# CelestineAngla/BundleAdjustment.jl

Hardware: AMD Instinct MI355X
Metric: LM iterations/sec on BAL venice-1778 (synthetic BAL-shaped), plus Jacobian Mnnz/sec (higher is better)
Workload: dtype f64; 1 GPU; venice-1778 shape: ncams=1778 npnts=993923 nobs=5001946, seed 20261004, lm.jl variant, LDL/None, facto_type f64, fixed 83 iterations, perm AMD; parallelism=points sharded over 1 rank(s), cameras replicated

## Files before the change

### bundleadjustment.jl_amd/csrc/ba_dense_ldl.hip

```cpp
#include "ba_internal.h"

#include <algorithm>
#include <atomic>
#include <cmath>
#include <cstdio>
#include <cstdlib>

namespace {

template <typename T>
struct RT;
template <>
struct RT<double> {
  typedef double v4 __attribute__((ext_vector_type(4)));
  typedef double v2 __attribute__((ext_vector_type(2)));
  static __device__ inline v4 mfma(double a, double b, v4 c) { return __builtin_amdgcn_mfma_f64_16x16x4f64(a, b, c, 0, 0, 0); }
  static __device__ inline int row(int lane, int reg) { return (lane >> 4) + 4 * reg; }
};
template <>
struct RT<float> {
  typedef float v4 __attribute__((ext_vector_type(4)));
  typedef float v2 __attribute__((ext_vector_type(2)));
  static __device__ inline v4 mfma(float a, float b, v4 c) { return __builtin_amdgcn_mfma_f32_16x16x4f32(a, b, c, 0, 0, 0); }
  static __device__ inline int row(int lane, int reg) { return 4 * (lane >> 4) + reg; }
// ... 965 lines not shown
    const int col = wc + 16 * n + (lane & 15);
    const T inv_d = (T)1 / Dk[col];
#pragma unroll
    for (int m = 0; m < 4; m++)
#pragma unroll
      for (int g = 0; g < 4; g++) {
        const int row = wr + 16 * m + RT<T>::row(lane, g);
        const T xv = acc[m][n][g];
        V10[row * NB + col] = xv;
        S10[row * NB + col] = xv * inv_d;
      }
  }
  __threadfence();
  __syncthreads();
  if (FWD) {
    if (tid < NB) {
      T sacc = 0;
      for (int c = 0; c < NB; c++) sacc += S10[tid * NB + c] * ysh[c];
      b[(int64_t)(k + 1) * NB + tid] -= sacc;
    }
  }
#pragma unroll
  for (int m = 0; m < 4; m++)
#pragma unroll
    for (int n = 0; n < 4; n++) acc[m][n] = (d4){0, 0, 0, 0};
  tile_gemm_abt<T, 1>(V10, S10, nullptr, nullptr, sm, sm + NB * LDK, acc);
#pragma unroll
  for (int n = 0; n < 4; n++) {
    const int col = wc + 16 * n + (lane & 15);
#pragma unroll
    for (int m = 0; m < 4; m++)
#pragma unroll
      for (int g = 0; g < 4; g++) {
        const int row = wr + 16 * m + RT<T>::row(lane, g);
        S11[row * NB + col] -= acc[m][n][g];
      }
  }
  __threadfence();
  __syncthreads();
  T *Lk1 = Lk + NB * NB, *Dk1 = Dk + NB;
  diag_tile<T, 4>(S11, Lk1, Dk1, flag, nullptr, sm);
  if (FWD) {
    __threadfence();
    __syncthreads();
    if (tid < NB) {
      T sacc = 0;
      for (int c = 0; c <= tid; c++) sacc += Lk1[tid * NB + c] * b[(int64_t)(k + 1) * NB + c];
      y[(int64_t)(k + 1) * NB + tid] = sacc;
    }
  }
}

template <typename T>
__device__ __forceinline__ void ldl_update_tile(T *__restrict__ S, const int64_t *__restrict__ co, const T *__restrict__ V0, const T *__restrict__ V1,
                                       int k, int i, int j, T *lds, const T *__restrict__ Lp0, const T *__restrict__ Lp1) {
  BA_VT
  T *Sij = S + tix(co, i, j) * NB * NB;
  typename RT<T>::v4 acc[4][4];
#pragma unroll
  for (int m = 0; m < 4; m++)
#pragma unroll
    for (int n = 0; n < 4; n++) acc[m][n] = (d4){0, 0, 0, 0};
  tile_gemm_abt_priv<T, 2>(V0 + (int64_t)i * NB * NB, Lp0 ? Lp0 + (int64_t)j * NB * NB : S + tix(co, j, k) * NB * NB,
                        V1 + (int64_t)i * NB * NB, Lp1 ? Lp1 + (int64_t)j * NB * NB : S + tix(co, j, k + 1) * NB * NB, lds, acc);
  int tid2 = threadIdx.x;
  asm volatile("" : "+v"(tid2));
  const int lane = tid2 & 63, wv = (tid2 >> 6) & 3;
  const int wr = (wv >> 1) * 64, wc = (wv & 1) * 64;
  T *cbase = Sij + wr * NB + wc + (lane & 15);
#pragma unroll
  for (int h = 0; h < 2; h++) {
    T cv[2][4][4];
#pragma unroll
    for (int n2 = 0; n2 < 2; n2++)
#pragma unroll
      for (int m = 0; m < 4; m++)
#pragma unroll
        for (int g = 0; g < 4; g++) cv[n2][m][g] = cbase[(16 * m + RT<T>::row(lane, g)) * NB + 16 * (2 * h + n2)];
#pragma unroll
    for (int n2 = 0; n2 < 2; n2++)
#pragma unroll
      for (int m = 0; m < 4; m++)
#pragma unroll
        for (int g = 0; g < 4; g++) {
          const T nv = cv[n2][m][g] - acc[m][2 * h + n2][g];
          cbase[(16 * m + RT<T>::row(lane, g)) * NB + 16 * (2 * h + n2)] = nv;
        }
  }
}

template <typename T, int MODE, bool OWN = false>
__global__ __launch_bounds__(256, 2) void k_ldl_update(T *__restrict__ S, const int64_t *__restrict__ co, const T *__restrict__ V0,
                                                        const T *__restrict__ V1, int k, int base, int nt,
                                                        int nblk, int *__restrict__ ready,
                                                        const int *__restrict__ own_cols = nullptr,
                                                        const int64_t *__restrict__ own_pref = nullptr, int m0 = 0,
                                                        int m_end = 0, int ready_tiles = 1, const int *__restrict__ rows = nullptr,
                                                        const T *__restrict__ Lp0 = nullptr, const T *__restrict__ Lp1 = nullptr,
                                                        const int2 *__restrict__ tlist = nullptr, int blocked = TSB) {
  BA_VT
  static_assert(MODE == 1, "only the pair update is a tile-per-workgroup kernel");
  extern __shared__ __attribute__((aligned(16))) unsigned char smraw[];
  T *lds = reinterpret_cast<T *>(smraw);
  int i, j, tsel;
  {
    const int per = (nblk + 7) / 8;
    int t = (blockIdx.x & 7) * per + (blockIdx.x >> 3);
    if (t >= nblk) return;
    tsel = t;
    if (tlist) {
      i = tlist[t].x;
      j = tlist[t].y;
    } else if (OWN) {
      const int64_t tt = t + own_pref[m0];
      int lo = m0, hi = m_end;
      while (hi - lo > 1) {
        const int mid = (lo + hi) >> 1;
        if (own_pref[mid] <= tt) lo = mid;
        else hi = mid;
      }
      j = own_cols[lo];
      i = j + (int)(tt - own_pref[lo]);
    } else {
      int m_rows = (int)((sqrt(8.0 * (double)nblk + 1.0) - 1.0) * 0.5);
      while ((m_rows + 1) * (m_rows + 2) / 2 <= nblk) m_rows++;
      while (m_rows * (m_rows + 1) / 2 > nblk) m_rows--;
      int ii, jj;
      if (blocked) {
        tri_blocked(t, m_rows, &ii, &jj, blocked);
      } else {
        ii = (int)((sqrt(8.0 * (double)t + 1.0) - 1.0) * 0.5);
        while ((ii + 1) * (ii + 2) / 2 <= t) ii++;
        while (ii * (ii + 1) / 2 > t) ii--;
        jj = t - ii * (ii + 1) / 2;
      }
      i = rows ? rows[ii] : base + ii;
      j = rows ? rows[jj] : base + jj;
    }
  }
  ldl_update_tile<T>(S, co, V0, V1, k, i, j, lds, Lp0, Lp1);
  if (ready && tsel < ready_tiles) {
    __threadfence();
    __syncthreads();
    if (threadIdx.x == 0) __hip_atomic_fetch_add(ready, 1, __ATOMIC_RELEASE, __HIP_MEMORY_SCOPE_AGENT);
  }
}

template <typename T>
constexpr size_t part_lds_bytes() { return 2 * gemm_priv_lds_bytes<T>(); }
template <typename T>
__global__ __launch_bounds__(512) void k_ldl_update_part(T *__restrict__ S, const int64_t *__restrict__ co, const T *__restrict__ V0,
                                                          const T *__restrict__ V1, int k, int nblk, const int *__restrict__ rows) {
  extern __shared__ __attribute__((aligned(16))) unsigned char smraw[];
  const int half = __builtin_amdgcn_readfirstlane((int)(threadIdx.x >> 8));
  T *lds = reinterpret_cast<T *>(smraw + half * gemm_priv_lds_bytes<T>());
  for (int t = 2 * blockIdx.x + half; t < nblk; t += 2 * gridDim.x) {
    int ii = (int)((sqrt(8.0 * (double)t + 1.0) - 1.0) * 0.5);
    while ((ii + 1) * (ii + 2) / 2 <= t) ii++;
    while (ii * (ii + 1) / 2 > t) ii--;
    const int jj = t - ii * (ii + 1) / 2;
    ldl_update_tile<T>(S, co, V0, V1, k, rows[ii], rows[jj], lds, nullptr, nullptr);
  }
}

template <typename T>
__global__ __launch_bounds__(512) void k_ldl_update_part2(T *__restrict__ S, const int64_t *__restrict__ co, RunPanel<T> a, int nblk_a,
                                                           RunPanel<T> c, int nblk_c, int64_t panel) {
  extern __shared__ __attribute__((aligned(16))) unsigned char smraw[];
  const int half = __builtin_amdgcn_readfirstlane((int)(threadIdx.x >> 8));
  T *lds = reinterpret_cast<T *>(smraw + half * gemm_priv_lds_bytes<T>());
  for (int tt = 2 * blockIdx.x + half; tt < nblk_a + nblk_c; tt += 2 * gridDim.x) {
    const bool second = tt >= nblk_a;
    const RunPanel<T> &r = second ? c : a;
    const int t = tt - (second ? nblk_a : 0);
    int ii = (int)((sqrt(8.0 * (double)t + 1.0) - 1.0) * 0.5);
    while ((ii + 1) * (ii + 2) / 2 <= t) ii++;
    while (ii * (ii + 1) / 2 > t) ii--;
    const int jj = t - ii * (ii + 1) / 2;
    ldl_update_tile<T>(S, co, r.V, r.V + panel, r.k, r.rows[ii], r.rows[jj], lds, nullptr, nullptr);
  }
}

template <typename T>
__global__ __launch_bounds__(256, 2) void k_ldl_update2(T *__restrict__ S, const int64_t *__restrict__ co, RunPanel<T> a, int nblk_a,
                                                         RunPanel<T> c, int nblk_c, int64_t panel) {
  extern __shared__ __attribute__((aligned(16))) unsigned char smraw[];
  T *lds = reinterpret_cast<T *>(smraw);
  const int ga = ((nblk_a + 7) / 8) * 8;
  const bool second = (int)blockIdx.x >= ga;
  const RunPanel<T> &r = second ? c : a;
  const int nblk = second ? nblk_c : nblk_a, bid = (int)blockIdx.x - (second ? ga : 0);
  const int per = (nblk + 7) / 8;
  const int t = (bid & 7) * per + (bid >> 3);
  if (t >= nblk) return;
  int ii = (int)((sqrt(8.0 * (double)t + 1.0) - 1.0) * 0.5);
  while ((ii + 1) * (ii + 2) / 2 <= t) ii++;
  while (ii * (ii + 1) / 2 > t) ii--;
  const int jj = t - ii * (ii + 1) / 2;
  ldl_update_tile<T>(S, co, r.V, r.V + panel, r.k, r.rows[ii], r.rows[jj], lds, nullptr, nullptr);
}

template <typename T>
__global__ __launch_bounds__(256) void k_ldl_scale_panel(T *__restrict__ Lcol, const T *__restrict__ V, const T *__restrict__ D_k, int i0,
                                                          const int *__restrict__ rows = nullptr) {
  BA_VT
  const int i = rows ? rows[blockIdx.x] : i0 + blockIdx.x;
  const T *Vi = V + (int64_t)i * NB * NB;
  T *Sik = Lcol + (int64_t)i * NB * NB;
  const int c2 = threadIdx.x & 63;
  const T inv0 = (T)1 / D_k[2 * c2], inv1 = (T)1 / D_k[2 * c2 + 1];
  for (int r = threadIdx.x >> 6; r < NB; r += 4) {
    d2 v = *reinterpret_cast<const d2 *>(Vi + r * NB + 2 * c2);
    v.x *= inv0;
    v.y *= inv1;
// ... 254 lines not shown
  col_off->assign((size_t)nt, 0);
  if (own_range) own_range->assign((size_t)world + 1, 0);
  int64_t off = 0;
  for (int r = 0; r < world; r++) {
    if (own_range) (*own_range)[(size_t)r] = off;
    for (int64_t q = r; 2 * q < nt; q += world)
      for (int64_t j = 2 * q; j < 2 * q + 2 && j < nt; j++) {
        (*col_off)[(size_t)j] = off;
        off += nt - j;
      }
  }
  if (own_range) (*own_range)[(size_t)world] = off;
}

template <typename T>
int dense_ldl_alloc(DenseLDLT<T> *w, int64_t n_unpadded, int world, int rank, bool lazy_S, bool own_only) {
  int64_t nt = (n_unpadded + NB - 1) / NB;
  if (nt < 1) nt = 1;
  w->n = nt * NB;
  w->nt = nt;
  w->world = world;
  w->rank = rank;
  dense_ldl_layout(nt, world, &w->h_glob_off, &w->own_range);
  w->h_col_tab.assign((size_t)nt + 1, 0);
  for (int64_t j = 0; j < nt; j++) w->hco()[j] = w->h_glob_off[(size_t)j];
  w->own_only = own_only && world > 1;
  w->s_tiles = nt * (nt + 1) / 2;
  if (w->own_only) {
    const int64_t base = w->own_range[(size_t)rank];
    for (int64_t j = 0; j < nt; j++)
      w->hco()[j] = ((j / 2) % world == rank) ? w->hco()[j] - base : BA_NO_TILE;
    w->s_tiles = std::max<int64_t>(1, w->own_range[(size_t)rank + 1] - base);
  }
  BA_CHECK(upload(w->col_tab, w->h_col_tab));
  w->col_off = w->col_tab + 1;
  w->h_own_cols.clear();
  w->h_own_pref.assign(1, 0);
  for (int64_t j = 0; j < nt; j++)
    if ((j / 2) % world == rank) {
      w->h_own_cols.push_back((int)j);
      w->h_own_pref.push_back(w->h_own_pref.back() + (nt - j));
    }
  BA_CHECK(upload(w->own_cols, w->h_own_cols, 1));
  BA_CHECK(upload(w->own_pref, w->h_own_pref));
  BA_CHECK(w->flag_sum.alloc(1));
  if (!lazy_S) BA_CHECK(dense_ldl_alloc_S(w));
  BA_CHECK(w->ev_chain.create(hipEventDisableTiming | hipEventReleaseToDevice));
  BA_CHECK(w->Linv.alloc(nt * NB * NB));
  BA_HIP_CHECK(hipMemset(w->Linv, 0, (size_t)nt * NB * NB * sizeof(T)));
  BA_HIP_CHECK(hipDeviceSynchronize());
  BA_CHECK(w->D.alloc(nt * NB * 2));
  BA_CHECK(w->flag.alloc(1));
  BA_CHECK(w->ready.alloc(nt));
  BA_CHECK(w->hoist.create(hipStreamNonBlocking));
  {
    int lo = 0, hi = 0;
    BA_HIP_CHECK(hipDeviceGetStreamPriorityRange(&lo, &hi));
    BA_CHECK(w->rest.create(hipStreamNonBlocking, lo));
  }
  BA_CHECK(w->ev_top.create(hipEventDisableTiming | hipEventReleaseToDevice));
  BA_CHECK(w->ev_dtop.create(hipEventDisableTiming));
  BA_CHECK(w->ev_dchain.create(hipEventDisableTiming));
  for (int q = 0; q < 2; q++) {
    BA_CHECK(w->ev_recv[q].create(hipEventDisableTiming));
    BA_CHECK(w->ev_upd[q].create(hipEventDisableTiming));
  }
  return set_kernel_attrs<T>();
}

template <typename T>
int dense_ldl_alloc_S(DenseLDLT<T> *w) {
  if (!w->S) BA_CHECK(w->S.alloc(w->s_tiles * NB * NB));
  if (!w->V) BA_CHECK(w->V.alloc(8 * w->nt * NB * NB));
  if (!w->Lb && w->own_only) BA_CHECK(w->Lb.alloc(4 * w->nt * NB * NB));
  if (!w->bpart && w->own_only) BA_CHECK(w->bpart.alloc(2 * w->nt * NB));
  return BA_OK;
}

struct PairRows {
  int k, c1, c2;
  const int *rows1, *rows2;
  const int *h_rows1;
  int row(int a) const { return h_rows1 ? h_rows1[a] : k + 1 + a; }
};

template <typename T>
static PairRows pair_rows(const DenseLDLT<T> *w, int q) {
  PairRows r = {2 * q, 0, 0, nullptr, nullptr, nullptr};
  if (const TilePattern *pat = w->pat) {
    const int l0 = pat->prow_ptr[(size_t)q];
    r.c1 = pat->prow_ptr[(size_t)q + 1] - l0;
    r.rows1 = w->prow + l0;
    r.rows2 = r.rows1 + 1;
    r.h_rows1 = pat->prow.data() + l0;
  } else {
    r.c1 = std::max(0, (int)w->nt - r.k - 1);
  }
  r.c2 = r.c1 > 0 ? r.c1 - 1 : 0;
  return r;
}

template <typename T>
static int launch_diag(ba_problem *p, DenseLDLT<T> *w, int k, hipStream_t st, const int *wait_ready = nullptr, bool clear_flag = false) {
  ProfScope ps(p, PC_LDL_DIAG, st);
  hipLaunchKernelGGL(k_ldl_diag<T>, dim3(1), dim3(DIAG_THREADS), DIAG_LDS_ELEMS * sizeof(T), st, w->S + tix(w->hco(), k, k) * NB * NB,
                     w->Linv + (int64_t)k * NB * NB, w->D + (int64_t)k * NB, w->flag, (unsigned long long *)nullptr,
                     wait_ready, clear_flag ? 1 : 0);
  return BA_OK;
}

template <typename K>
static K fwd_kernel(const void *b, K with_fwd, K without) { return b ? with_fwd : without; }

template <typename T>
static int launch_trsm(ba_problem *p, DenseLDLT<T> *w, int k, const int *rows, int count, T *V, T *b, hipStream_t st) {
  T *y = w->D + w->nt * NB;
  if (count <= 0) {
    if (b) hipLaunchKernelGGL(k_fwd_step<T>, dim3(1), dim3(256), 0, st, w->S, w->col_off, w->Linv, b, y, k);
    return BA_OK;
  }
  ProfScope ps(p, PC_LDL_TRSM, st);
  hipLaunchKernelGGL(fwd_kernel(b, k_ldl_trsm_rs<T, true>, k_ldl_trsm_rs<T, false>), dim3(4 * count), dim3(256), RS_LDS_ELEMS * sizeof(T),
                     st, w->S, w->col_off, w->Linv + (int64_t)k * NB * NB, w->D + (int64_t)k * NB, V, k, b, y, rows);
  return BA_OK;
}

template <typename T>
static int launch_col(ba_problem *p, DenseLDLT<T> *w, int k, const int *rows, int count, const T *V0, hipStream_t st) {
  if (count <= 0) return BA_OK;
  ProfScope ps(p, PC_LDL_SYRK, st);
  hipLaunchKernelGGL(k_ldl_col_rs<T>, dim3(4 * count), dim3(256), RS_LDS_ELEMS * sizeof(T), st, w->S, w->col_off, V0, k, rows);
  return BA_OK;
}

static int update_rs_max() {
  return env_int("BA_LDL_UPDATE_RS_MAX", 320);
}

template <typename T>
static int launch_pair(ba_problem *p, DenseLDLT<T> *w, int k, const int *rows, int count, const T *V0, const T *V1, hipStream_t st,
                       int *ready = nullptr, int ready_tiles = 1) {
  const int nblk = count * (count + 1) / 2;
  if (nblk <= 0) return BA_OK;
  if (!ready && nblk <= update_rs_max()) {
    ProfScope ps(p, PC_LDL_UPDATE_RS, st);
    hipLaunchKernelGGL(k_ldl_update_rs<T>, dim3(4 * nblk), dim3(256), RS_LDS_ELEMS * sizeof(T), st, w->S, w->col_off, V0, V1, k, k + 2, nblk,
                       rows);
    return BA_OK;
  }
  ProfScope ps(p, PC_LDL_UPDATE, st);
  hipLaunchKernelGGL((k_ldl_update<T, 1>), dim3(((nblk + 7) / 8) * 8), dim3(256), gemm_priv_lds_bytes<T>(), st, w->S,
                     w->col_off, V0, V1, k, k + 2, (int)w->nt, nblk, ready, (const int *)nullptr, (const int64_t *)nullptr, 0, 0,
                     ready_tiles, rows);
  return BA_OK;
}

template <typename T>
static int launch_pairdiag(ba_problem *p, DenseLDLT<T> *w, int k, T *V0, T *b, hipStream_t st, const int *wait_ready, int need) {
  ProfScope ps(p, PC_LDL_DIAG, st);
  T *y = w->D + w->nt * NB;
  hipLaunchKernelGGL(fwd_kernel(b, k_ldl_pairdiag<T, true>, k_ldl_pairdiag<T, false>), dim3(1), dim3(256), DIAG_LDS_ELEMS * sizeof(T), st,
                     w->S, w->col_off, w->Linv, w->D, V0, k, (int)w->nt, w->flag, wait_ready, need, b, y);
  return BA_OK;
}

template <typename T>
static int launch_pairtrsm(ba_problem *p, DenseLDLT<T> *w, int k, T *V0, T *V1, T *b, hipStream_t st) {
  const int m = (int)w->nt - k - 2;
  if (m <= 0) return BA_OK;
  ProfScope ps(p, PC_LDL_TRSM, st);
  const T *y = w->D + w->nt * NB;
  hipLaunchKernelGGL(fwd_kernel(b, k_ldl_pairtrsm<T, true>, k_ldl_pairtrsm<T, false>), dim3(4 * m), dim3(256), PT_LDS_ELEMS * sizeof(T), st,
                     w->S, w->col_off, w->Linv, w->D, V0, V1, k, b, y);
  return BA_OK;
}

template <typename T>
static int panel_chain(ba_problem *p, DenseLDLT<T> *w, const PairRows &r, T *V0, T *V1, T *b, hipStream_t st) {
  launch_trsm(p, w, r.k, r.rows1, r.c1, V0, b, st);
  if (r.c1 == 0) return BA_OK;
  launch_col(p, w, r.k, r.rows1, r.c1, V0, st);
  launch_diag(p, w, r.k + 1, st);
  launch_trsm(p, w, r.k + 1, r.rows2, r.c2, V1, b, st);
  return BA_OK;
}

template <typename T>
int dense_ldl_factor_sparse(ba_problem *p, DenseLDLT<T> *w, hipStream_t st, T *d_b);

template <typename T>
int dense_ldl_factor(ba_problem *p, DenseLDLT<T> *w, hipStream_t st, T *d_b) {
  if (w->sparse && !p->comm.active()) return dense_ldl_factor_sparse(p, w, st, d_b);
  const int nt = (int)w->nt;
  static const bool hoist_off = env_off("BA_LDL_HOIST");
  w->hoisting = !p->prof_on && !hoist_off && !w->hoist_disabled && !p->comm.active() && nt >= HOIST_MIN_TILES + 2 && nt <= HOIST_MAX_TILES;
  if (w->hoisting) {
    BA_HIP_CHECK(hipMemsetAsync(w->flag, 0, sizeof(int), st));
    BA_HIP_CHECK(hipMemsetAsync(w->ready, 0, (size_t)nt * sizeof(int), st));
    BA_HIP_CHECK(hipEventRecord(w->ev_top, st));
    BA_HIP_CHECK(hipStreamWaitEvent(w->hoist, w->ev_top, 0));
  }
  constexpr int FUSE_MIN_TILES = 48;
  static const bool fuse_off = env_off("BA_LDL_FUSE");
  auto fused = [&](int k) { return w->hoisting && !fuse_off && k >= 2 && k + 1 < nt && nt - k >= FUSE_MIN_TILES; };
  launch_diag(p, w, 0, st, nullptr, !w->hoisting);
  for (int k = 0, slot = 0; k < nt; k += 2, slot ^= 1) {
    const PairRows r = pair_rows(w, k / 2);
    T *V0 = w->vpanel(slot, 0), *V1 = w->vpanel(slot, 1);
    const bool more = k + 2 < nt;
    const bool next_fused = more && fused(k + 2);
    const bool next_hoist1 = more && !next_fused && w->hoisting && (nt - k - 2 >= HOIST_MIN_TILES);
    const int need = (k + 3 < nt) ? 3 : 1;
    if (next_fused) {
      launch_pairdiag(p, w, k + 2, w->vpanel(slot ^ 1, 0), d_b, w->hoist, w->ready + k + 2, need);
      BA_HIP_CHECK(hipEventRecord(w->ev_chain, w->hoist));
    } else if (next_hoist1) {
      launch_diag(p, w, k + 2, w->hoist, w->ready + k + 2);
      BA_HIP_CHECK(hipEventRecord(w->ev_chain, w->hoist));
    }
    if (fused(k)) launch_pairtrsm(p, w, k, V0, V1, d_b, st);
    else panel_chain(p, w, r, V0, V1, d_b, st);
    if (!more) break;
    const bool hoisted = next_fused || next_hoist1;
    launch_pair(p, w, k, r.rows2, r.c2, V0, V1, st, hoisted ? w->ready + k + 2 : nullptr, next_fused ? need : 1);
    if (hoisted)
      BA_HIP_CHECK(hipStreamWaitEvent(st, w->ev_chain, 0));
    else
      launch_diag(p, w, k + 2, st);
  }
  BA_HIP_CHECK(hipGetLastError());
  return BA_OK;
}


template <typename T>
int dense_ldl_use_pattern(DenseLDLT<T> *w, const TilePattern *pat) {
  for (DevBuf<int> *q : {&w->prow, &w->lcol, &w->lpair}) q->reset();
  w->upd_ij.reset();
  w->own_tiles.reset();
  w->pat = pat;
  w->sparse = pat != nullptr;
  if (!pat) return BA_OK;
  {
    const int64_t nt = w->nt;
    const int P = w->own_only ? w->world : 1, me = w->own_only ? w->rank : 0;
    std::vector<int64_t> tab((size_t)(1 + nt + nt * nt), BA_NO_TILE);
    tab[0] = nt;
    int64_t *co = tab.data() + 1, *rp = tab.data() + 1 + nt;
    w->h_col_cnt.assign((size_t)nt, 0);
    for (int64_t j = 0; j < nt; j++) {
      const int64_t q = j / 2;
      int64_t pos = 0;
      rp[j * nt + j] = pos++;
      const int l0 = pat->prow_ptr[(size_t)q], l1 = pat->prow_ptr[(size_t)q + 1];
      for (int l = l0; l < l1; l++) {
        const int64_t i = pat->prow[(size_t)l];
        if (i > j) rp[i * nt + j] = pos++;
      }
      w->h_col_cnt[(size_t)j] = pos;
    }
    w->own_range.assign((size_t)P + 1, 0);
    int64_t run = 0;
    for (int r = 0; r < P; r++) {
      w->own_range[(size_t)r] = run;
      for (int64_t j = 0; j < nt; j++)
        if ((j / 2) % P == r) {
          if (r == me) co[j] = run;
          run += w->h_col_cnt[(size_t)j];
        }
    }
    w->own_range[(size_t)P] = run;
    const int64_t base = w->own_range[(size_t)me];
    for (int64_t j = 0; j < nt; j++)
      if (co[j] >= 0) co[j] -= base;
    w->s_tiles = std::max<int64_t>(1, w->own_range[(size_t)me + 1] - base);
    if (w->own_only) {
      w->h_own_pref.assign(1, 0);
      std::vector<int2> tiles;
      for (int j : w->h_own_cols) {
        w->h_own_pref.push_back(w->h_own_pref.back() + w->h_col_cnt[(size_t)j]);
        const int64_t q = j / 2;
        tiles.push_back(make_int2(j, j));
        for (int l = pat->prow_ptr[(size_t)q]; l < pat->prow_ptr[(size_t)q + 1]; l++)
          if (pat->prow[(size_t)l] > j) tiles.push_back(make_int2(pat->prow[(size_t)l], j));
      }
      BA_HIP_CHECK(hipMemcpy(w->own_pref, w->h_own_pref.data(), w->h_own_pref.size() * sizeof(int64_t), hipMemcpyHostToDevice));
      BA_CHECK(upload(w->own_tiles, tiles, 1));
      std::vector<int2> upd;
      const int npairs = (int)((nt + 1) / 2);
      w->h_upd_ptr.assign(1, 0);
      w->h_upd_lead.assign((size_t)npairs, 0);
      for (int q = 0; q < npairs; q++) {
        const int k = 2 * q, l0 = pat->prow_ptr[(size_t)q], l1 = pat->prow_ptr[(size_t)q + 1];
        for (int a = l0 + 1; a < l1; a++) {
          const int j = pat->prow[(size_t)a];
          if ((j / 2) % P != me) continue;
          for (int c = a; c < l1; c++) upd.push_back(make_int2(pat->prow[(size_t)c], j));
          if (j < k + 4) w->h_upd_lead[(size_t)q] = (int)upd.size() - w->h_upd_ptr.back();
        }
        w->h_upd_ptr.push_back((int)upd.size());
      }
      BA_CHECK(upload(w->upd_ij, upd, 1));
    }
    w->h_col_tab.swap(tab);
    BA_CHECK(upload(w->col_tab, w->h_col_tab));
    w->col_off = w->col_tab + 1;
    if (w->S) BA_CHECK(w->S.alloc(w->s_tiles * NB * NB));
  }
  BA_CHECK(upload(w->prow, pat->prow, 1));
  BA_CHECK(upload(w->lcol, pat->lcol, 1));
  BA_CHECK(upload(w->lpair, pat->lpair, 1));
  return BA_OK;
}

constexpr int REST_CUS = 224;
static int rest_grid(int ntile) { return (ntile + 1) / 2 < REST_CUS ? (ntile + 1) / 2 : REST_CUS; }

struct UpdateSplit {
  int nlead, lead_tiles, rest_tiles;
};
static UpdateSplit update_split(const PairRows &r) {
  int nlead = 0;
  while (nlead < r.c2 && nlead < 2 && r.row(1 + nlead) < r.k + 4) nlead++;
  const int nrest = r.c2 - nlead;
  return {nlead, nlead == 0 ? 0 : (nlead == 1 ? r.c2 : 2 * r.c2 - 1), nrest * (nrest + 1) / 2};
}

template <typename T>
int dense_ldl_factor_sparse(ba_problem *p, DenseLDLT<T> *w, hipStream_t st, T *d_b) {
  const int nt = (int)w->nt;
  const TilePattern *pat = w->pat;
  const int64_t panel = (int64_t)nt * NB * NB;
  const int npairs = (nt + 1) / 2;
  T *y = w->D + w->nt * NB;
  w->hoisting = false;
  const bool lookahead = !p->prof_on && !env_off("BA_SPARSE_LOOKAHEAD");
  const int la_min = env_int("BA_SPARSE_LOOKAHEAD_MIN", 96);
  bool pending[2] = {false, false};
  auto join_rest = [&](int slot) -> int {
    if (pending[slot]) {
      BA_HIP_CHECK(hipStreamWaitEvent(st, w->ev_upd[slot], 0));
      pending[slot] = false;
    }
    return BA_OK;
  };
  auto fork_rest = [&](int slot) -> int {
    BA_HIP_CHECK(hipEventRecord(w->ev_recv[slot], st));
    BA_HIP_CHECK(hipStreamWaitEvent(w->rest, w->ev_recv[slot], 0));
    return BA_OK;
  };
  auto rest_launched = [&](int slot) -> int {
    BA_HIP_CHECK(hipEventRecord(w->ev_upd[slot], w->rest));
    pending[slot] = true;
    return BA_OK;
  };
  const bool two = pat->a_clean > 0 && pat->b_clean > 0 && !p->prof_on && !env_off("BA_SPARSE_TWO_RUNS");
  std::vector<int> order;
  if (two) {
    BA_HIP_CHECK(hipMemsetAsync(w->flag, 0, sizeof(int), st));
    const int both = std::min(pat->a_clean, pat->b_clean);
    for (int i = 0; i < both; i++) {
      const int slot = i & 1;
      const PairRows a = pair_rows(w, i), b = pair_rows(w, pat->split + i);
      T *VA = w->vpanel(slot, 0, 0), *VB = w->vpanel(slot, 0, 1);
      auto tile = [&](int k) { return w->S + tix(w->hco(), k, k) * NB * NB; };
      auto panel_of = [&](int k, T *V, const int *rows) { return RunPanel<T>{w->Linv + (int64_t)k * NB * NB, w->D + (int64_t)k * NB, V, k, rows}; };
      auto diag2 = [&](int ka, int kb) {
        hipLaunchKernelGGL(k_ldl_diag2<T>, dim3(2), dim3(DIAG_THREADS), DIAG_LDS_ELEMS * sizeof(T), st, tile(ka), w->Linv + (int64_t)ka * NB * NB,
                           w->D + (int64_t)ka * NB, tile(kb), w->Linv + (int64_t)kb * NB * NB, w->D + (int64_t)kb * NB, w->flag);
      };
      auto trsm2 = [&](const RunPanel<T> &pa, int ca, const RunPanel<T> &pb, int cb) {
        hipLaunchKernelGGL(fwd_kernel(d_b, k_ldl_trsm_rs2<T, true>, k_ldl_trsm_rs2<T, false>), dim3(4 * (ca + cb)), dim3(256),
                           RS_LDS_ELEMS * sizeof(T), st, w->S, w->col_off, pa, pb, 4 * ca, d_b, y);
      };
      BA_CHECK(join_rest(slot));
      diag2(a.k, b.k);
      const RunPanel<T> a0 = panel_of(a.k, VA, a.rows1), b0 = panel_of(b.k, VB, b.rows1);
      trsm2(a0, a.c1, b0, b.c1);
      hipLaunchKernelGGL(k_ldl_col_rs2<T>, dim3(4 * (a.c1 + b.c1)), dim3(256), RS_LDS_ELEMS * sizeof(T), st, w->S, w->col_off, a0, b0, 4 * a.c1);
      diag2(a.k + 1, b.k + 1);
      trsm2(panel_of(a.k + 1, VA + panel, a.rows2), a.c2, panel_of(b.k + 1, VB + panel, b.rows2), b.c2);
      const UpdateSplit sa = update_split(a), sb = update_split(b);
      const RunPanel<T> ua = panel_of(a.k, VA, a.rows2), ub = panel_of(b.k, VB, b.rows2);
      BA_CHECK(join_rest(slot ^ 1));
      if (lookahead && i + 1 < both && sa.rest_tiles + sb.rest_tiles >= 2 * la_min) {
        if (sa.lead_tiles + sb.lead_tiles > 0)
          hipLaunchKernelGGL(k_ldl_update_rs2<T>, dim3(4 * (sa.lead_tiles + sb.lead_tiles)), dim3(256), RS_LDS_ELEMS * sizeof(T), st, w->S, w->col_off,
                             ua, sa.lead_tiles, ub, sb.lead_tiles, panel, a.c2, b.c2);
        BA_CHECK(fork_rest(slot));
        hipLaunchKernelGGL(k_ldl_update_part2<T>, dim3(rest_grid(sa.rest_tiles + sb.rest_tiles)), dim3(512), part_lds_bytes<T>(), w->rest, w->S, w->col_off,
                           panel_of(a.k, VA, a.rows2 + sa.nlead), sa.rest_tiles, panel_of(b.k, VB, b.rows2 + sb.nlead), sb.rest_tiles, panel);
        BA_CHECK(rest_launched(slot));
      } else {
        const int na = a.c2 * (a.c2 + 1) / 2, nb2 = b.c2 * (b.c2 + 1) / 2;
        if (na + nb2 <= update_rs_max())
          hipLaunchKernelGGL(k_ldl_update_rs2<T>, dim3(4 * (na + nb2)), dim3(256), RS_LDS_ELEMS * sizeof(T), st, w->S, w->col_off, ua, na, ub, nb2, panel, 0, 0);
        else
          hipLaunchKernelGGL(k_ldl_update2<T>, dim3(((na + 7) / 8) * 8 + ((nb2 + 7) / 8) * 8), dim3(256), gemm_priv_lds_bytes<T>(), st, w->S, w->col_off,
                             ua, na, ub, nb2, panel);
      }
    }
    BA_CHECK(join_rest(0));
    BA_CHECK(join_rest(1));
    BA_HIP_CHECK(hipGetLastError());
    for (int q = both; q < pat->a_clean; q++) order.push_back(q);
    for (int q = pat->a_clean; q < pat->split; q++) order.push_back(q);
    for (int q = pat->split + both; q < npairs; q++) order.push_back(q);
  } else {
    for (int q = 0; q < npairs; q++) order.push_back(q);
  }
  for (size_t it = 0; it < order.size(); it++) {
    const PairRows r = pair_rows(w, order[it]);
    const int slot = (int)(it & 1);
    T *V0 = w->vpanel(slot, 0), *V1 = w->vpanel(slot, 1);
    BA_CHECK(join_rest(slot));
    launch_diag(p, w, r.k, st, nullptr, !two && r.k == 0);
    panel_chain(p, w, r, V0, V1, d_b, st);
    if (r.c2 == 0) continue;
    const bool next_adjacent = it + 1 < order.size() && order[it + 1] == order[it] + 1;
    const UpdateSplit s = update_split(r);
    BA_CHECK(join_rest(slot ^ 1));
    if (lookahead && next_adjacent && s.rest_tiles >= la_min) {
      if (s.nlead > 0) {
        ProfScope ps(p, PC_LDL_UPDATE_RS, st);
        hipLaunchKernelGGL(k_ldl_update_rs<T>, dim3(4 * s.lead_tiles), dim3(256), RS_LDS_ELEMS * sizeof(T), st, w->S, w->col_off, V0, V1, r.k,
                           r.k + 2, s.lead_tiles, r.rows2, r.c2);
      }
      BA_CHECK(fork_rest(slot));
      hipLaunchKernelGGL(k_ldl_update_part<T>, dim3(rest_grid(s.rest_tiles)), dim3(512), part_lds_bytes<T>(), w->rest, w->S, w->col_off, V0, V1,
                         r.k, s.rest_tiles, r.rows2 + s.nlead);
      BA_CHECK(rest_launched(slot));
    } else {
      launch_pair(p, w, r.k, r.rows2, r.c2, V0, V1, st);
    }
  }
  BA_CHECK(join_rest(0));
  BA_CHECK(join_rest(1));
  BA_HIP_CHECK(hipGetLastError());
  return BA_OK;
}

template <typename T>
static int launch_pair_owned(ba_problem *p, DenseLDLT<T> *w, int k, const T *V0, const T *V1, hipStream_t st, int m0, int m1) {
  if (m0 >= m1) return BA_OK;
  const int64_t nblk64 = w->h_own_pref[(size_t)m1] - w->h_own_pref[(size_t)m0];
  if (nblk64 <= 0) return BA_OK;
  const int nblk = (int)nblk64;
  ProfScope ps(p, PC_LDL_UPDATE, st);
  const T *Lp0 = nullptr, *Lp1 = nullptr;
  if (w->own_only) {
    Lp0 = w->L_of(V0);
    Lp1 = w->L_of(V1);
  }
  hipLaunchKernelGGL((k_ldl_update<T, 1, true>), dim3(((nblk + 7) / 8) * 8), dim3(256), gemm_priv_lds_bytes<T>(), st,
                     w->S, w->col_off, V0, V1, k, w->h_own_cols[(size_t)m0], (int)w->nt, nblk, (int *)nullptr, w->own_cols, w->own_pref, m0, m1,
                     1, (const int *)nullptr, Lp0, Lp1);
  return BA_OK;
}

template <typename T>
static int launch_pair_list(ba_problem *p, DenseLDLT<T> *w, int q, const T *V0, const T *V1, hipStream_t st, int from, int to) {
  const int nblk = to - from;
  if (nblk <= 0) return BA_OK;
  ProfScope ps(p, PC_LDL_UPDATE, st);
  hipLaunchKernelGGL((k_ldl_update<T, 1>), dim3(((nblk + 7) / 8) * 8), dim3(256), gemm_priv_lds_bytes<T>(), st, w->S, w->col_off, V0, V1,
                     2 * q, 2 * q + 2, (int)w->nt, nblk, (int *)nullptr, (const int *)nullptr, (const int64_t *)nullptr, 0, 0, 1,
                     (const int *)nullptr, w->L_of(V0), w->L_of(V1), (const int2 *)(w->upd_ij + w->h_upd_ptr[(size_t)q] + from));
  return BA_OK;
}

template <typename T>
static int dist_chain(ba_problem *p, DenseLDLT<T> *w, int k, T *V0, T *V1, hipStream_t st) {
  launch_diag(p, w, k, st);
  panel_chain(p, w, pair_rows(w, k / 2), V0, V1, (T *)nullptr, st);
  BA_HIP_CHECK(hipGetLastError());
  return BA_OK;
}

template <typename T>
static void launch_scale_panel(DenseLDLT<T> *w, T *Lcol, const T *V, int c, const int *rows, int count, hipStream_t st) {
  if (count > 0) hipLaunchKernelGGL(k_ldl_scale_panel<T>, dim3(count), dim3(256), 0, st, Lcol, V, w->D + (int64_t)c * NB, c + 1, rows);
}

template <typename T>
static int dist_transfer(ba_problem *p, DenseLDLT<T> *w, int k, T *V0, T *V1, int owner, hipStream_t st) {
  const bool two = k + 1 < (int)w->nt;
  const PairRows r = pair_rows(w, k / 2);
  BA_CHECK(comm_group_begin(p));
  int rc = BA_OK;
  auto bcast_rows = [&](T *V, int first, int cnt) {
// ... 413 lines not shown
```

### bundleadjustment.jl_amd/csrc/ba_internal.h

```cpp
#pragma once
#include <hip/hip_runtime.h>
#include <stdint.h>
#include <stdlib.h>
#include <string>
#include <vector>

#include "../../include/ba_hip.h"
#include "ba_order.h"

void ba_set_error(const char *fmt, ...);

#define BA_HIP_CHECK(expr)                                                                          \
  do {                                                                                              \
    hipError_t _e = (expr);                                                                         \
    if (_e != hipSuccess) {                                                                         \
      ba_set_error("%s:%d: %s -> %s", __FILE__, __LINE__, #expr, hipGetErrorString(_e));            \
      return BA_ERR_HIP;                                                                            \
    }                                                                                               \
  } while (0)

#define BA_CHECK(expr)            \
  do {                            \
    int _rc = (expr);             \
    if (_rc != BA_OK) return _rc; \
// ... 63 lines not shown
class HipStream : public Owner<hipStream_t, hipStreamDestroy> {
 public:
  int create(unsigned flags) {
    BA_HIP_CHECK(hipStreamCreateWithFlags(out(), flags));
    return BA_OK;
  }
  int create(unsigned flags, int priority) {
    BA_HIP_CHECK(hipStreamCreateWithPriority(out(), flags, priority));
    return BA_OK;
  }
};
class HipEvent : public Owner<hipEvent_t, hipEventDestroy> {
 public:
  int create(unsigned flags = hipEventDefault) {
    BA_HIP_CHECK(hipEventCreateWithFlags(out(), flags));
    return BA_OK;
  }
};
using HipGraph = Owner<hipGraph_t, hipGraphDestroy>;
using HipGraphExec = Owner<hipGraphExec_t, hipGraphExecDestroy>;

template <typename T>
int upload(DevBuf<T> &d, const std::vector<T> &h, size_t extra = 0) {
  BA_CHECK(d.alloc((int64_t)(h.size() + extra)));
  if (!h.empty()) BA_HIP_CHECK(hipMemcpy(d, h.data(), h.size() * sizeof(T), hipMemcpyHostToDevice));
  return BA_OK;
}

constexpr int NB = 128;
constexpr int TSB = 8;
__host__ __device__ inline void tri_blocked(int t, int m, int *ii, int *jj, int sb = TSB) {
  const int full = sb * sb, tri = sb * (sb + 1) / 2;
  int lo = 0, hi = (m + sb - 1) / sb;
  while (hi - lo > 1) {
    const int mid = (lo + hi) >> 1;
    if (full * mid * (mid - 1) / 2 + tri * mid <= t) lo = mid;
    else hi = mid;
  }
  const int bi = lo;
  int rem = t - (full * bi * (bi - 1) / 2 + tri * bi);
  const int h = (m - sb * bi) < sb ? (m - sb * bi) : sb;
  if (rem < bi * sb * h) {
    const int bj = rem / (sb * h), r2 = rem - bj * (sb * h);
    *ii = sb * bi + r2 / sb;
    *jj = sb * bj + r2 % sb;
  } else {
    rem -= bi * sb * h;
    int r = 0;
    while ((r + 1) * (r + 2) / 2 <= rem) r++;
    *ii = sb * bi + r;
    *jj = sb * bi + rem - r * (r + 1) / 2;
  }
}

__host__ __device__ inline int64_t tix(const int64_t *__restrict__ col_off, int64_t i, int64_t j) {
  const int64_t n = col_off[-1];
  return col_off[j] + (n ? col_off[n + i * n + j] : (i - j));
}
constexpr int64_t BA_NO_TILE = -((int64_t)1 << 40);
void dense_ldl_layout(int64_t nt, int world, std::vector<int64_t> *col_off, std::vector<int64_t> *own_range);

enum ProfClass {
  PC_RESIDUAL = 0,
  PC_JAC_STRUCTURE,
  PC_JAC_COORD,
  PC_POINT_BLOCKS,
  PC_CAM_BLOCKS,
  PC_SCHUR_PREP,
  PC_SCHUR_S,
  PC_SCHUR_RHS,
  PC_LDL_DIAG,
  PC_LDL_TRSM,
  PC_LDL_SYRK,
  PC_LDL_UPDATE,
  PC_LDL_UPDATE_RS,
  PC_SOLVE,
  PC_BACKSUB,
  PC_TRIAL,
  PC_REDUCE,
  PC_COMM,
  PC_ROBUST,
  PC_FIXED,
  PC_COV_INV,
  PC_COV_CAMS,
  PC_COV_POINTS,
  PC_PRIOR,
  PC_SHARED_BORDER,
  PC_SHARED_SWEEP,
  PC_SHARED_SMALL,
  PC_COUNT
};
extern const char *const kProfNames[PC_COUNT];

struct ProfSlot {
  double ms = 0;
  int64_t calls = 0;
};

template <typename T>
struct DenseLDLT {
  int64_t n = 0, nt = 0;
  DevBuf<T> S;
  DevBuf<T> V;
  T *vpanel(int slot, int j, int run = 0) { return V + (int64_t)(4 * run + 2 * slot + j) * nt * NB * NB; }
  DevBuf<T> Linv;
  DevBuf<T> D;
  int64_t *col_off = nullptr;
  std::vector<int64_t> h_col_tab;
  DevBuf<int64_t> col_tab;
  const int64_t *hco() const { return h_col_tab.data() + 1; }
  int64_t *hco() { return h_col_tab.data() + 1; }
  std::vector<int64_t> own_range;
  int world = 1, rank = 0;
  std::vector<int> h_own_cols;
  std::vector<int64_t> h_own_pref;
  DevBuf<int> own_cols;
  DevBuf<int64_t> own_pref;
  DevBuf<double> flag_sum;
  DevBuf<int> flag;
  DevBuf<int> ready;
  HipStream hoist;
  HipStream rest;
  HipEvent ev_top;
  bool hoist_disabled = false;
  bool hoisting = false;
  HipEvent ev_chain;
  HipEvent ev_recv[2], ev_upd[2];
  bool own_only = false;
  int64_t s_tiles = 0;
  std::vector<int64_t> h_glob_off;
  DevBuf<T> Lb, bpart;
  T *L_of(const T *v) { return Lb + (v - V); }
  bool sparse = false;
  const TilePattern *pat = nullptr;
  DevBuf<int> prow, lcol, lpair;
  std::vector<int64_t> h_col_cnt;
  std::vector<int> h_upd_ptr, h_upd_lead;
  DevBuf<int2> upd_ij, own_tiles;
  HipEvent ev_dtop, ev_dchain;
};
typedef DenseLDLT<double> DenseLDL;
constexpr int HOIST_MIN_TILES = 32;
constexpr int HOIST_MAX_TILES = 224;

struct BaComm {
  int rank = 0, world = 1;
  ba_comm_fn hook = nullptr;
  void *hook_ctx = nullptr;
  void *nccl = nullptr;
  int64_t calls = 0, bytes = 0;
  int64_t op_calls[BA_COMM_OPS] = {}, op_bytes[BA_COMM_OPS] = {};
  bool active() const { return hook != nullptr || nccl != nullptr; }
};

void lm_free(ba_problem *p);

struct PriorSet {
  int64_t n = 0;
  std::vector<int> h_idx;
  std::vector<double> h_mu, h_info;
  DevBuf<int> idx;
  DevBuf<double> mu, info;
};
enum { PRI_PNT = 0, PRI_CAM, PRI_CTR, PRI_KINDS };

struct ba_problem {
  int device = 0;
  HipStream stream;
  int64_t ncams = 0, npnts = 0, nobs = 0;
  DevBuf<int> cam0, pnt0;
  DevBuf<double> pt2d;
  DevBuf<float> pt2d_f32;
  DevBuf<int> pt_ptr, pt_obs;
// ... 95 lines not shown
```

Measured before the change: 27.99 LM iterations/s.

## Add persistent ticket-based tile scheduling and tail lookahead for dense LDL updates

The dense LDL pair-update kernel becomes a persistent grid, sized to the CU count, that pulls tiles from per-XCD atomic ticket queues. Ready tiles are served first, and a workgroup steals from other queues once its own runs dry. The next ticket is drawn while the current tile's writeback is in progress, to overlap scheduling with compute. Separately, tail iterations of the dense factorization split the update into lead tiles on the main stream and the remaining tiles on a side stream (lookahead reused from the sparse path), so the next diagonal/trsm can start early. This adds atomics, extra syncthreads and cross-stream event overhead.

New measurement: 28.44 LM iterations/s (median of 6 runs). 1.6% higher.

```diff
diff --git a/bundleadjustment.jl_amd/csrc/ba_dense_ldl.hip b/bundleadjustment.jl_amd/csrc/ba_dense_ldl.hip
--- a/bundleadjustment.jl_amd/csrc/ba_dense_ldl.hip
+++ b/bundleadjustment.jl_amd/csrc/ba_dense_ldl.hip
@@ -1041,8 +1041,9 @@
 }
 
 template <typename T>
-__device__ __forceinline__ void ldl_update_tile(T *__restrict__ S, const int64_t *__restrict__ co, const T *__restrict__ V0, const T *__restrict__ V1,
-                                       int k, int i, int j, T *lds, const T *__restrict__ Lp0, const T *__restrict__ Lp1) {
+__device__ __forceinline__ int ldl_update_tile(T *__restrict__ S, const int64_t *__restrict__ co, const T *__restrict__ V0, const T *__restrict__ V1,
+                                      int k, int i, int j, T *lds, const T *__restrict__ Lp0, const T *__restrict__ Lp1,
+                                      int *__restrict__ ticket = nullptr) {
   BA_VT
   T *Sij = S + tix(co, i, j) * NB * NB;
   typename RT<T>::v4 acc[4][4];
@@ -1054,6 +1055,8 @@
                         V1 + (int64_t)i * NB * NB, Lp1 ? Lp1 + (int64_t)j * NB * NB : S + tix(co, j, k + 1) * NB * NB, lds, acc);
   int tid2 = threadIdx.x;
   asm volatile("" : "+v"(tid2));
+  int drawn = 0;
+  if (ticket && tid2 == 0) drawn = __hip_atomic_fetch_add(ticket, 1, __ATOMIC_RELAXED, __HIP_MEMORY_SCOPE_AGENT);
   const int lane = tid2 & 63, wv = (tid2 >> 6) & 3;
   const int wr = (wv >> 1) * 64, wc = (wv & 1) * 64;
   T *cbase = Sij + wr * NB + wc + (lane & 15);
@@ -1076,6 +1079,7 @@
           cbase[(16 * m + RT<T>::row(lane, g)) * NB + 16 * (2 * h + n2)] = nv;
         }
   }
+  return drawn;
 }
 
 template <typename T, int MODE, bool OWN = false>
@@ -1086,11 +1090,61 @@
                                                         const int64_t *__restrict__ own_pref = nullptr, int m0 = 0,
                                                         int m_end = 0, int ready_tiles = 1, const int *__restrict__ rows = nullptr,
                                                         const T *__restrict__ Lp0 = nullptr, const T *__restrict__ Lp1 = nullptr,
-                                                        const int2 *__restrict__ tlist = nullptr, int blocked = TSB) {
+                                                        const int2 *__restrict__ tlist = nullptr, int blocked = TSB,
+                                                        int *__restrict__ tickets = nullptr) {
   BA_VT
   static_assert(MODE == 1, "only the pair update is a tile-per-workgroup kernel");
   extern __shared__ __attribute__((aligned(16))) unsigned char smraw[];
   T *lds = reinterpret_cast<T *>(smraw);
+  if constexpr (!OWN) {
+    if (tickets) {
+      __shared__ int s_next[2], s_src[2];
+      int m_rows = (int)((sqrt(8.0 * (double)nblk + 1.0) - 1.0) * 0.5);
+      while ((m_rows + 1) * (m_rows + 2) / 2 <= nblk) m_rows++;
+      while (m_rows * (m_rows + 1) / 2 > nblk) m_rows--;
+      const int nready = ready ? ready_tiles : 0;
+      const int xcd = (int)(__builtin_amdgcn_s_getreg(20 | (0 << 6) | ((4 - 1) << 11)) & (TICKET_QUEUES - 1));
+      const bool wave0 = __builtin_amdgcn_readfirstlane((int)(threadIdx.x >> 6)) == 0;
+      auto take = [&](int src, int drawn, int slot) {
+        const bool first = (threadIdx.x & 63) == 0;
+        int n_raw = __builtin_amdgcn_readfirstlane(drawn), t;
+        for (;;) {
+          t = ticket_tile(nblk, nready, ticket_source(xcd, src), n_raw);
+          if (t >= 0 || src == TICKET_QUEUES) break;
+          src++;
+          int v = 0;
+          if (first) v = __hip_atomic_fetch_add(tickets + ticket_source(xcd, src), 1, __ATOMIC_RELAXED, __HIP_MEMORY_SCOPE_AGENT);
+          n_raw = __builtin_amdgcn_readfirstlane(v);
+        }
+        if (first) {
+          s_next[slot] = t;
+          s_src[slot] = src;
+        }
+      };
+      if (wave0) {
+        int v = 0;
+        if (threadIdx.x == 0) v = __hip_atomic_fetch_add(tickets + TICKET_READY, 1, __ATOMIC_RELAXED, __HIP_MEMORY_SCOPE_AGENT);
+        take(0, v, 0);
+      }
+      const int sb = blocked > 0 ? blocked : TSB;
+      for (int par = 0;; par ^= 1) {
+        __syncthreads();
+        const int t = __builtin_amdgcn_readfirstlane(s_next[par]);
+        if (t < 0) return;
+        const int src = __builtin_amdgcn_readfirstlane(s_src[par]);
+        int ii, jj;
+        tri_blocked(t, m_rows, &ii, &jj, sb);
+        const int n_raw = ldl_update_tile<T>(S, co, V0, V1, k, rows ? rows[ii] : base + ii, rows ? rows[jj] : base + jj, lds, Lp0, Lp1,
+                                             tickets + ticket_source(xcd, src));
+        if (ready && t < ready_tiles) {
+          __threadfence();
+          __syncthreads();
+          if (threadIdx.x == 0) __hip_atomic_fetch_add(ready, 1, __ATOMIC_RELEASE, __HIP_MEMORY_SCOPE_AGENT);
+        }
+        if (wave0) take(src, n_raw, par ^ 1);
+      }
+    }
+  }
   int i, j, tsel;
   {
     const int per = (nblk + 7) / 8;
@@ -1139,7 +1193,8 @@
 constexpr size_t part_lds_bytes() { return 2 * gemm_priv_lds_bytes<T>(); }
 template <typename T>
 __global__ __launch_bounds__(512) void k_ldl_update_part(T *__restrict__ S, const int64_t *__restrict__ co, const T *__restrict__ V0,
-                                                          const T *__restrict__ V1, int k, int nblk, const int *__restrict__ rows) {
+                                                          const T *__restrict__ V1, int k, int nblk, const int *__restrict__ rows,
+                                                          int base) {
   extern __shared__ __attribute__((aligned(16))) unsigned char smraw[];
   const int half = __builtin_amdgcn_readfirstlane((int)(threadIdx.x >> 8));
   T *lds = reinterpret_cast<T *>(smraw + half * gemm_priv_lds_bytes<T>());
@@ -1148,7 +1203,7 @@
     while ((ii + 1) * (ii + 2) / 2 <= t) ii++;
     while (ii * (ii + 1) / 2 > t) ii--;
     const int jj = t - ii * (ii + 1) / 2;
-    ldl_update_tile<T>(S, co, V0, V1, k, rows[ii], rows[jj], lds, nullptr, nullptr);
+    ldl_update_tile<T>(S, co, V0, V1, k, rows ? rows[ii] : base + ii, rows ? rows[jj] : base + jj, lds, nullptr, nullptr);
   }
 }
 
@@ -1509,6 +1564,13 @@
   BA_CHECK(w->D.alloc(nt * NB * 2));
   BA_CHECK(w->flag.alloc(1));
   BA_CHECK(w->ready.alloc(nt));
+  BA_CHECK(w->tickets.alloc((nt / 2 + 1) * TICKET_SLOTS));
+  {
+    int dev = 0, cus = 0;
+    BA_HIP_CHECK(hipGetDevice(&dev));
+    BA_HIP_CHECK(hipDeviceGetAttribute(&cus, hipDeviceAttributeMultiprocessorCount, dev));
+    w->wg_slots = 2 * std::max(cus, 1);
+  }
   BA_CHECK(w->hoist.create(hipStreamNonBlocking));
   {
     int lo = 0, hi = 0;
@@ -1596,7 +1658,7 @@
 
 template <typename T>
 static int launch_pair(ba_problem *p, DenseLDLT<T> *w, int k, const int *rows, int count, const T *V0, const T *V1, hipStream_t st,
-                       int *ready = nullptr, int ready_tiles = 1) {
+                       int *ready = nullptr, int ready_tiles = 1, int *tickets = nullptr) {
   const int nblk = count * (count + 1) / 2;
   if (nblk <= 0) return BA_OK;
   if (!ready && nblk <= update_rs_max()) {
@@ -1606,9 +1668,10 @@
     return BA_OK;
   }
   ProfScope ps(p, PC_LDL_UPDATE, st);
-  hipLaunchKernelGGL((k_ldl_update<T, 1>), dim3(((nblk + 7) / 8) * 8), dim3(256), gemm_priv_lds_bytes<T>(), st, w->S,
+  const int grid = tickets ? std::min(std::max(w->wg_slots - (ready ? 2 : 0), 1), nblk) : ((nblk + 7) / 8) * 8;
+  hipLaunchKernelGGL((k_ldl_update<T, 1>), dim3(grid), dim3(256), gemm_priv_lds_bytes<T>(), st, w->S,
                      w->col_off, V0, V1, k, k + 2, (int)w->nt, nblk, ready, (const int *)nullptr, (const int64_t *)nullptr, 0, 0,
-                     ready_tiles, rows);
+                     ready_tiles, rows, (const T *)nullptr, (const T *)nullptr, (const int2 *)nullptr, TSB, tickets);
   return BA_OK;
 }
 
@@ -1640,6 +1703,59 @@
   launch_diag(p, w, r.k + 1, st);
   launch_trsm(p, w, r.k + 1, r.rows2, r.c2, V1, b, st);
   return BA_OK;
+}
+
+constexpr int REST_CUS = 224;
+constexpr int TAIL_REST_CUS = 192, TAIL_AHEAD_MIN_TILES = 96;
+static int rest_grid(int ntile, int cus = REST_CUS) { return (ntile + 1) / 2 < cus ? (ntile + 1) / 2 : cus; }
+
+struct UpdateSplit {
+  int nlead, lead_tiles, rest_tiles;
+};
+static UpdateSplit update_split(const PairRows &r) {
+  int nlead = 0;
+  while (nlead < r.c2 && nlead < 2 && r.row(1 + nlead) < r.k + 4) nlead++;
+  const int nrest = r.c2 - nlead;
+  return {nlead, nlead == 0 ? 0 : (nlead == 1 ? r.c2 : 2 * r.c2 - 1), nrest * (nrest + 1) / 2};
+}
+
+
+template <typename T>
+struct RestAhead {
+  DenseLDLT<T> *w;
+  hipStream_t st;
+  bool pending[2] = {false, false};
+  int join(int slot) {
+    if (pending[slot]) {
+      BA_HIP_CHECK(hipStreamWaitEvent(st, w->ev_upd[slot], 0));
+      pending[slot] = false;
+    }
+    return BA_OK;
+  }
+  int fork(int slot) {
+    BA_HIP_CHECK(hipEventRecord(w->ev_recv[slot], st));
+    BA_HIP_CHECK(hipStreamWaitEvent(w->rest, w->ev_recv[slot], 0));
+    return BA_OK;
+  }
+  int launched(int slot) {
+    BA_HIP_CHECK(hipEventRecord(w->ev_upd[slot], w->rest));
+    pending[slot] = true;
+    return BA_OK;
+  }
+};
+
+template <typename T>
+static int launch_pair_ahead(ba_problem *p, DenseLDLT<T> *w, RestAhead<T> &la, const PairRows &r, const UpdateSplit &s, int slot, const T *V0,
+                             const T *V1, int rest_cus) {
+  if (s.nlead > 0) {
+    ProfScope ps(p, PC_LDL_UPDATE_RS, la.st);
+    hipLaunchKernelGGL(k_ldl_update_rs<T>, dim3(4 * s.lead_tiles), dim3(256), RS_LDS_ELEMS * sizeof(T), la.st, w->S, w->col_off, V0, V1, r.k,
+                       r.k + 2, s.lead_tiles, r.rows2, r.c2);
+  }
+  BA_CHECK(la.fork(slot));
+  hipLaunchKernelGGL(k_ldl_update_part<T>, dim3(rest_grid(s.rest_tiles, rest_cus)), dim3(512), part_lds_bytes<T>(), w->rest, w->S, w->col_off, V0,
+                     V1, r.k, s.rest_tiles, r.rows2 ? r.rows2 + s.nlead : nullptr, r.k + 2 + s.nlead);
+  return la.launched(slot);
 }
 
 template <typename T>
@@ -1660,14 +1776,23 @@
   constexpr int FUSE_MIN_TILES = 48;
   static const bool fuse_off = env_off("BA_LDL_FUSE");
   auto fused = [&](int k) { return w->hoisting && !fuse_off && k >= 2 && k + 1 < nt && nt - k >= FUSE_MIN_TILES; };
+  const bool tickets_on = !env_off("BA_LDL_TICKETS") && (nt - 2) * (nt - 1) / 2 > update_rs_max();
+  if (tickets_on) BA_HIP_CHECK(hipMemsetAsync(w->tickets, 0, (size_t)(nt / 2 + 1) * TICKET_SLOTS * sizeof(int), st));
+  const bool tail_ahead = !p->prof_on && !p->comm.active() && !hoist_off && !w->hoist_disabled && !(w->hoisting && fuse_off) &&
+                          !env_off("BA_LDL_TAIL_LOOKAHEAD");
+  const int ahead_min = env_int("BA_LDL_TAIL_LOOKAHEAD_MIN", TAIL_AHEAD_MIN_TILES);
+  RestAhead<T> la{w, st};
   launch_diag(p, w, 0, st, nullptr, !w->hoisting);
   for (int k = 0, slot = 0; k < nt; k += 2, slot ^= 1) {
     const PairRows r = pair_rows(w, k / 2);
     T *V0 = w->vpanel(slot, 0), *V1 = w->vpanel(slot, 1);
     const bool more = k + 2 < nt;
     const bool next_fused = more && fused(k + 2);
-    const bool next_hoist1 = more && !next_fused && w->hoisting && (nt - k - 2 >= HOIST_MIN_TILES);
+    const UpdateSplit s = update_split(r);
+    const bool ahead = tail_ahead && more && !fused(k) && !next_fused && nt - k < FUSE_MIN_TILES && s.rest_tiles >= std::max(ahead_min, 1);
+    const bool next_hoist1 = more && !next_fused && !ahead && w->hoisting && (nt - k - 2 >= HOIST_MIN_TILES);
     const int need = (k + 3 < nt) ? 3 : 1;
+    BA_CHECK(la.join(slot));
     if (next_fused) {
       launch_pairdiag(p, w, k + 2, w->vpanel(slot ^ 1, 0), d_b, w->hoist, w->ready + k + 2, need);
       BA_HIP_CHECK(hipEventRecord(w->ev_chain, w->hoist));
@@ -1678,13 +1803,20 @@
     if (fused(k)) launch_pairtrsm(p, w, k, V0, V1, d_b, st);
     else panel_chain(p, w, r, V0, V1, d_b, st);
     if (!more) break;
+    BA_CHECK(la.join(slot ^ 1));
     const bool hoisted = next_fused || next_hoist1;
-    launch_pair(p, w, k, r.rows2, r.c2, V0, V1, st, hoisted ? w->ready + k + 2 : nullptr, next_fused ? need : 1);
+    if (ahead)
+      BA_CHECK(launch_pair_ahead(p, w, la, r, s, slot, V0, V1, TAIL_REST_CUS));
+    else
+      launch_pair(p, w, k, r.rows2, r.c2, V0, V1, st, hoisted ? w->ready + k + 2 : nullptr, next_fused ? need : 1,
+                  tickets_on ? w->tickets + (k / 2) * TICKET_SLOTS : nullptr);
     if (hoisted)
       BA_HIP_CHECK(hipStreamWaitEvent(st, w->ev_chain, 0));
     else
       launch_diag(p, w, k + 2, st);
   }
+  BA_CHECK(la.join(0));
+  BA_CHECK(la.join(1));
   BA_HIP_CHECK(hipGetLastError());
   return BA_OK;
 }
@@ -1770,19 +1902,6 @@
   return BA_OK;
 }
 
-constexpr int REST_CUS = 224;
-static int rest_grid(int ntile) { return (ntile + 1) / 2 < REST_CUS ? (ntile + 1) / 2 : REST_CUS; }
-
-struct UpdateSplit {
-  int nlead, lead_tiles, rest_tiles;
-};
-static UpdateSplit update_split(const PairRows &r) {
-  int nlead = 0;
-  while (nlead < r.c2 && nlead < 2 && r.row(1 + nlead) < r.k + 4) nlead++;
-  const int nrest = r.c2 - nlead;
-  return {nlead, nlead == 0 ? 0 : (nlead == 1 ? r.c2 : 2 * r.c2 - 1), nrest * (nrest + 1) / 2};
-}
-
 template <typename T>
 int dense_ldl_factor_sparse(ba_problem *p, DenseLDLT<T> *w, hipStream_t st, T *d_b) {
   const int nt = (int)w->nt;
@@ -1793,24 +1912,7 @@
   w->hoisting = false;
   const bool lookahead = !p->prof_on && !env_off("BA_SPARSE_LOOKAHEAD");
   const int la_min = env_int("BA_SPARSE_LOOKAHEAD_MIN", 96);
-  bool pending[2] = {false, false};
-  auto join_rest = [&](int slot) -> int {
-    if (pending[slot]) {
-      BA_HIP_CHECK(hipStreamWaitEvent(st, w->ev_upd[slot], 0));
-      pending[slot] = false;
-    }
-    return BA_OK;
-  };
-  auto fork_rest = [&](int slot) -> int {
-    BA_HIP_CHECK(hipEventRecord(w->ev_recv[slot], st));
-    BA_HIP_CHECK(hipStreamWaitEvent(w->rest, w->ev_recv[slot], 0));
-    return BA_OK;
-  };
-  auto rest_launched = [&](int slot) -> int {
-    BA_HIP_CHECK(hipEventRecord(w->ev_upd[slot], w->rest));
-    pending[slot] = true;
-    return BA_OK;
-  };
+  RestAhead<T> la{w, st};
   const bool two = pat->a_clean > 0 && pat->b_clean > 0 && !p->prof_on && !env_off("BA_SPARSE_TWO_RUNS");
   std::vector<int> order;
   if (two) {
@@ -1830,7 +1932,7 @@
         hipLaunchKernelGGL(fwd_kernel(d_b, k_ldl_trsm_rs2<T, true>, k_ldl_trsm_rs2<T, false>), dim3(4 * (ca + cb)), dim3(256),
                            RS_LDS_ELEMS * sizeof(T), st, w->S, w->col_off, pa, pb, 4 * ca, d_b, y);
       };
-      BA_CHECK(join_rest(slot));
+      BA_CHECK(la.join(slot));
       diag2(a.k, b.k);
       const RunPanel<T> a0 = panel_of(a.k, VA, a.rows1), b0 = panel_of(b.k, VB, b.rows1);
       trsm2(a0, a.c1, b0, b.c1);
@@ -1839,15 +1941,15 @@
       trsm2(panel_of(a.k + 1, VA + panel, a.rows2), a.c2, panel_of(b.k + 1, VB + panel, b.rows2), b.c2);
       const UpdateSplit sa = update_split(a), sb = update_split(b);
       const RunPanel<T> ua = panel_of(a.k, VA, a.rows2), ub = panel_of(b.k, VB, b.rows2);
-      BA_CHECK(join_rest(slot ^ 1));
+      BA_CHECK(la.join(slot ^ 1));
       if (lookahead && i + 1 < both && sa.rest_tiles + sb.rest_tiles >= 2 * la_min) {
         if (sa.lead_tiles + sb.lead_tiles > 0)
           hipLaunchKernelGGL(k_ldl_update_rs2<T>, dim3(4 * (sa.lead_tiles + sb.lead_tiles)), dim3(256), RS_LDS_ELEMS * sizeof(T), st, w->S, w->col_off,
                              ua, sa.lead_tiles, ub, sb.lead_tiles, panel, a.c2, b.c2);
-        BA_CHECK(fork_rest(slot));
+        BA_CHECK(la.fork(slot));
         hipLaunchKernelGGL(k_ldl_update_part2<T>, dim3(rest_grid(sa.rest_tiles + sb.rest_tiles)), dim3(512), part_lds_bytes<T>(), w->rest, w->S, w->col_off,
                            panel_of(a.k, VA, a.rows2 + sa.nlead), sa.rest_tiles, panel_of(b.k, VB, b.rows2 + sb.nlead), sb.rest_tiles, panel);
-        BA_CHECK(rest_launched(slot));
+        BA_CHECK(la.launched(slot));
       } else {
         const int na = a.c2 * (a.c2 + 1) / 2, nb2 = b.c2 * (b.c2 + 1) / 2;
         if (na + nb2 <= update_rs_max())
@@ -1857,8 +1959,8 @@
                              ua, na, ub, nb2, panel);
       }
     }
-    BA_CHECK(join_rest(0));
-    BA_CHECK(join_rest(1));
+    BA_CHECK(la.join(0));
+    BA_CHECK(la.join(1));
     BA_HIP_CHECK(hipGetLastError());
     for (int q = both; q < pat->a_clean; q++) order.push_back(q);
     for (int q = pat->a_clean; q < pat->split; q++) order.push_back(q);
@@ -1870,29 +1972,21 @@
     const PairRows r = pair_rows(w, order[it]);
     const int slot = (int)(it & 1);
     T *V0 = w->vpanel(slot, 0), *V1 = w->vpanel(slot, 1);
-    BA_CHECK(join_rest(slot));
+    BA_CHECK(la.join(slot));
     launch_diag(p, w, r.k, st, nullptr, !two && r.k == 0);
     panel_chain(p, w, r, V0, V1, d_b, st);
     if (r.c2 == 0) continue;
     const bool next_adjacent = it + 1 < order.size() && order[it + 1] == order[it] + 1;
     const UpdateSplit s = update_split(r);
-    BA_CHECK(join_rest(slot ^ 1));
+    BA_CHECK(la.join(slot ^ 1));
     if (lookahead && next_adjacent && s.rest_tiles >= la_min) {
-      if (s.nlead > 0) {
-        ProfScope ps(p, PC_LDL_UPDATE_RS, st);
-        hipLaunchKernelGGL(k_ldl_update_rs<T>, dim3(4 * s.lead_tiles), dim3(256), RS_LDS_ELEMS * sizeof(T), st, w->S, w->col_off, V0, V1, r.k,
-                           r.k + 2, s.lead_tiles, r.rows2, r.c2);
-      }
-      BA_CHECK(fork_rest(slot));
-      hipLaunchKernelGGL(k_ldl_update_part<T>, dim3(rest_grid(s.rest_tiles)), dim3(512), part_lds_bytes<T>(), w->rest, w->S, w->col_off, V0, V1,
-                         r.k, s.rest_tiles, r.rows2 + s.nlead);
-      BA_CHECK(rest_launched(slot));
+      BA_CHECK(launch_pair_ahead(p, w, la, r, s, slot, V0, V1, REST_CUS));
     } else {
       launch_pair(p, w, r.k, r.rows2, r.c2, V0, V1, st);
     }
   }
-  BA_CHECK(join_rest(0));
-  BA_CHECK(join_rest(1));
+  BA_CHECK(la.join(0));
+  BA_CHECK(la.join(1));
   BA_HIP_CHECK(hipGetLastError());
   return BA_OK;
 }
diff --git a/bundleadjustment.jl_amd/csrc/ba_internal.h b/bundleadjustment.jl_amd/csrc/ba_internal.h
--- a/bundleadjustment.jl_amd/csrc/ba_internal.h
+++ b/bundleadjustment.jl_amd/csrc/ba_internal.h
@@ -139,6 +139,18 @@
     *jj = sb * bi + rem - r * (r + 1) / 2;
   }
 }
+
+constexpr int TICKET_QUEUES = 8, TICKET_READY = TICKET_QUEUES;
+constexpr int TICKET_SLOTS = 16;
+__host__ __device__ inline int ticket_tile(int nblk, int ready_tiles, int src, int n) {
+  const int nready = ready_tiles < nblk ? ready_tiles : nblk;
+  if (src == TICKET_READY) return n < nready ? n : -1;
+  const int per = (nblk + TICKET_QUEUES - 1) / TICKET_QUEUES;
+  const int lo = src * per > nready ? src * per : nready;
+  const int hi = (src + 1) * per < nblk ? (src + 1) * per : nblk;
+  return n < hi - lo ? lo + n : -1;
+}
+__host__ __device__ inline int ticket_source(int xcd, int s) { return s == 0 ? TICKET_READY : (xcd + s - 1) % TICKET_QUEUES; }
 
 __host__ __device__ inline int64_t tix(const int64_t *__restrict__ col_off, int64_t i, int64_t j) {
   const int64_t n = col_off[-1];
@@ -206,6 +218,8 @@
   DevBuf<double> flag_sum;
   DevBuf<int> flag;
   DevBuf<int> ready;
+  DevBuf<int> tickets;
+  int wg_slots = 0;
   HipStream hoist;
   HipStream rest;
   HipEvent ev_top;
```
